# johanna-rock/quantization_analysis

Measured on AMD Instinct MI355X. Metric: 32x32 tiles/s for mixed-tile-greedy (bf16->BFP{8,4,2}); achieved HBM GB/s vs peak, higher is better.
Workload: dtype f32/f64

## Files before the change

### quantization_analysis_amd/csrc/mtq_fast.hip

```cpp
#include <hip/hip_runtime.h>
#include <stdint.h>
#include <stdlib.h>

#include "../../include/mtq.h"
#include "mtq_device.hpp"
#include "mtq_error.hpp"

namespace mtq {

typedef unsigned short us2 __attribute__((ext_vector_type(2)));
typedef short s2 __attribute__((ext_vector_type(2)));

__device__ __forceinline__ us2 as_us2(uint32_t x) { return __builtin_bit_cast(us2, x); }
__device__ __forceinline__ s2 as_s2(uint32_t x) { return __builtin_bit_cast(s2, x); }
__device__ __forceinline__ uint32_t as_u32(us2 x) { return __builtin_bit_cast(uint32_t, x); }
__device__ __forceinline__ uint32_t as_u32(s2 x) { return __builtin_bit_cast(uint32_t, x); }

#ifndef MTQ_FAST_WAVES
#define MTQ_FAST_WAVES 2
#endif
constexpr int kFastWaves = MTQ_FAST_WAVES;
constexpr int kUnitTiles = 4;
constexpr int kUnitCols = kUnitTiles * kTile;
constexpr int kInBytes = kTile * kUnitCols * 2;
// ... 315 lines not shown

__host__ __device__ constexpr int rolled_waves(uint32_t sums, uint32_t errs)
{
#ifdef MTQ_ROLLED_WAVES_PER_SIMD_FORCE
    return MTQ_ROLLED_WAVES_PER_SIMD_FORCE;
#elif defined(MTQ_K1_INTDOM)
    return (sums == 7u && errs == 7u) ? 3 : 4;
#else
    const uint32_t any = sums | errs;
    const int n = (int)((any & 1u) + ((any >> 1) & 1u) + ((any >> 2) & 1u));
    if (n >= 2) return 3;
    return errs == 0u ? 5 : 4;
#endif
}

struct PlaceArgs { uint32_t eval_mask; int o_bf16, o8, o4, o2; };
__device__ __forceinline__ void place_stat(const PlaceArgs pa, double *rec_t, int sidx, double r)
{
    if (sidx == 0) {
        rec_t[0] = r;
        if (pa.eval_mask & 1u) {
            const double z = __builtin_fabs(r) * 0.0;
            rec_t[pa.o_bf16] = r; rec_t[pa.o_bf16 + 3] = z; rec_t[pa.o_bf16 + 4] = z;
        }
    } else if (sidx == 1) {
        rec_t[1] = r;
        if (pa.eval_mask & 1u) { rec_t[pa.o_bf16 + 1] = r; rec_t[pa.o_bf16 + 2] = r; }
    } else {
        const int f = (sidx - 2) >> 2, k = (sidx - 2) & 3;
        const int o = f == 0 ? pa.o8 : (f == 1 ? pa.o4 : pa.o2);
        if (pa.eval_mask & (2u << f)) rec_t[o + k] = r;
    }
}

struct ListedArgs {
    const uint32_t *list, *n_list;
    uint32_t cap;
    uint32_t *redo, *n_redo;
    uint32_t tiles_w32;
};

template <uint32_t SUMS, uint32_t ERRS, bool XS, bool LISTED>
__global__ __launch_bounds__(kFastWaves * 64, rolled_waves(SUMS, ERRS)) void tile_stats_bf16_rolled(
    const uint16_t *__restrict__ x, int64_t stride, int64_t ld, int tiles_w, int64_t tiles, int units_w, int units_per_tensor,
    int total_units, uint32_t fmt_mask, uint32_t eval_mask, uint32_t part_mask, int rec, double *__restrict__ stats, unsigned *__restrict__ work,
    unsigned launch_id, int units_per_wave, ListedArgs la, unsigned *__restrict__ mark, int self_reset)
{
    constexpr int nsum = terms_needed(SUMS, ERRS, XS);
    constexpr int npass = (nsum + kPassMax - 1) / kPassMax, per = (nsum + npass - 1) / npass;
    constexpr int scratch_doubles = kUnitTiles * per * kScratchStride;
    static_assert((scratch_doubles + kRecDoubles) * 8 <= kHalfBytes, "reduce scratch + record image must fit in half the input image");
    extern __shared__ __attribute__((aligned(16))) unsigned char lds[];
    const int lane = threadIdx.x & 63;
    const int wave = __builtin_amdgcn_readfirstlane(threadIdx.x >> 6);
    unsigned char *in = lds + wave * kRolledWaveLds;
    const uint32_t in_addr = (uint32_t)(uintptr_t)(__attribute__((address_space(3))) unsigned char *)in;
    const uint32_t t = lane >> 4, j = lane & 15;

    uint32_t dma_off[8], dma_tile[8];
#pragma unroll
    for (int i = 0; i < 8; ++i) {
        const uint32_t rho = lane >> 4;
        const uint32_t c = (lane & 15u) ^ swz(4u * (i & 3) + rho);
        const uint32_t row = 8u * (i & 3) + 2u * rho + (uint32_t)(i >> 2);
        dma_off[i] = LISTED ? (uint32_t)(row * ld * 2) + (c & 3u) * 16u : (uint32_t)(row * ld * 2) + c * 16u;
        dma_tile[i] = c >> 2;
    }
    const uint32_t rd_row = j * 256u;
    const uint32_t c0 = (4u * t) ^ swz(j);

    const int groups = (int)min(gridDim.x, (unsigned)kWorkGroups), group = (int)(blockIdx.x % (unsigned)groups);
    unsigned *queue = LISTED ? nullptr : work + group * kWorkStride;
    uint32_t n_listed = 0u;
    if constexpr (LISTED) {
        n_listed = min(*la.n_list, la.cap);
        total_units = (int)((n_listed + 3u) >> 2);
    }
    int stride_next = (int)(blockIdx.x * kFastWaves) + wave;
    auto claim_first = [&]() -> int {
        if constexpr (LISTED) {
            const int u = stride_next;
            stride_next += (int)gridDim.x * kFastWaves;
// ... 32 lines not shown
    auto locate = [&](int u) -> Where {
        Where w{nullptr, nullptr, 0ull};
        if constexpr (LISTED) {
            const uint32_t gt = listed_tile(u, (uint32_t)lane & 3u);
            const uint32_t b = gt / (uint32_t)tiles, tt = gt - b * (uint32_t)tiles;
            const uint32_t tr = tt / la.tiles_w32, tc = tt - tr * la.tiles_w32;
            w.mine = (unsigned long long)(uintptr_t)(x + (int64_t)b * stride + ((int64_t)tr * kTile) * ld + (int64_t)tc * kTile);
        } else {
            const int b = u / units_per_tensor, r = u - b * units_per_tensor, tr = r / units_w, uc = r - tr * units_w;
            w.base = reinterpret_cast<const unsigned char *>(x + (int64_t)b * stride + ((int64_t)tr * kTile) * ld + (int64_t)uc * kUnitCols);
            w.out = stats + ((int64_t)b * tiles + (int64_t)tr * tiles_w + uc * kUnitTiles) * rec;
        }
        return w;
    };
    auto issue_rows = [&](const Where &w, int odd, uint32_t half) {
        if constexpr (LISTED) {
#pragma unroll
            for (int i = 0; i < 4; ++i) {
                const uint32_t tl = odd ? dma_tile[4 + i] : dma_tile[i], off = odd ? dma_off[4 + i] : dma_off[i];
                const unsigned lo = (unsigned)__shfl((int)(unsigned)w.mine, (int)tl, 64), hi = (unsigned)__shfl((int)(unsigned)(w.mine >> 32), (int)tl, 64);
                const unsigned long long src = (((unsigned long long)hi << 32) | lo) + off;
                glds16v(reinterpret_cast<const void *>((uintptr_t)src), half + i * 1024);
            }
        } else {
#pragma unroll
            for (int i = 0; i < 4; ++i) glds16(w.base, odd ? dma_off[4 + i] : dma_off[i], half + i * 1024);
        }
    };
    const PlaceArgs pa{eval_mask, o_bf16, o8, o4, o2};
    auto tree16 = [&](const double *row) -> double {
        double v[16];
#pragma unroll
        for (int k = 0; k < 16; ++k) v[k] = row[k];
#pragma unroll
        for (int stp = 1; stp < 16; stp <<= 1)
#pragma unroll
            for (int k = 0; k < 16; k += 2 * stp) v[k] = v[k] + v[k + stp];
        return v[0];
    };

    int left = units_per_wave > 0 ? units_per_wave : 0x7FFFFFFF;
// ... 245 lines not shown
```

### quantization_analysis_amd/csrc/mtq_scan.hip

```cpp
#include <hip/hip_runtime.h>
#include <stdint.h>

#include <atomic>
#include <type_traits>
#include <stdlib.h>
#include <mutex>

#include "../../include/mtq.h"
#include "mtq_decide.hpp"
#include "mtq_error.hpp"

namespace mtq {
namespace {

constexpr int kScanMaxTilesLds = 32768;
constexpr int kTagSlots = 16384;
constexpr int kJump = 34;

} }
__device__ unsigned long long g_scan_ticks[16];
namespace mtq { namespace {

struct U128 { uint64_t lo, hi; };
__host__ __device__ inline U128 mul128(U128 a, U128 b)
{
#if defined(__HIP_DEVICE_COMPILE__)
    const uint64_t h = __umul64hi(a.lo, b.lo);
#else
    const uint64_t h = (uint64_t)(((unsigned __int128)a.lo * b.lo) >> 64);
#endif
    return {a.lo * b.lo, h + a.lo * b.hi + a.hi * b.lo};
}
// ... 55 lines not shown
__device__ inline double ld_l2(const double *p) { return __longlong_as_double((long long)ld_l2(reinterpret_cast<const unsigned long long *>(p))); }
__device__ inline void mem_wait() { __builtin_amdgcn_s_waitcnt(0); __builtin_amdgcn_fence(__ATOMIC_ACQ_REL, "workgroup"); }

__device__ inline void compiler_fence() { asm volatile("" ::: "memory"); }
__device__ inline uint64_t below(int lane) { return lane >= 64 ? ~0ull : ((1ull << lane) - 1ull); }
__device__ inline double shfl_f64(double v, int src)
{
    const unsigned long long u = (unsigned long long)__double_as_longlong(v);
    const unsigned lo = (unsigned)__shfl((int)(unsigned)u, src, 64), hi = (unsigned)__shfl((int)(unsigned)(u >> 32), src, 64);
    return __longlong_as_double((long long)(((unsigned long long)hi << 32) | lo));
}

__device__ inline uint64_t readlane_u64(uint64_t u, int src)
{
    const unsigned lo = (unsigned)__builtin_amdgcn_readlane((int)(unsigned)u, src), hi = (unsigned)__builtin_amdgcn_readlane((int)(unsigned)(u >> 32), src);
    return ((uint64_t)hi << 32) | lo;
}

__device__ inline double readlane_f64(double v, int src) { return __longlong_as_double((long long)readlane_u64((uint64_t)__double_as_longlong(v), src)); }

struct OrderLds {
    uint16_t *p;
    __device__ uint32_t get(uint32_t i) const { return p[i]; }
    __device__ void set(uint32_t i, uint32_t v) const { p[i] = (uint16_t)v; }
    __device__ void sync() const { __builtin_amdgcn_s_waitcnt(0xC07F);  __builtin_amdgcn_fence(__ATOMIC_ACQ_REL, "workgroup"); }
    __device__ void sync_reads() const { compiler_fence(); }
    __device__ void sync_writes() const { compiler_fence(); }
};
struct OrderGlobal {
    uint32_t *p;
    __device__ uint32_t get(uint32_t i) const { return ld_l2(p + i); }
    __device__ void set(uint32_t i, uint32_t v) const { p[i] = v; }
    __device__ void sync() const { mem_wait(); }
    __device__ void sync_reads() const { mem_wait(); }
    __device__ void sync_writes() const { mem_wait(); }
};

struct Rng {
    U128 state;
    bool has32;
    uint32_t u32;
    U128 a0, c0, a1, c1;
};

#ifdef MTQ_SCAN_PROFILE
#define MTQ_SHUF_TICK(slot) do { const unsigned long long now_ = clock64(); if (blockIdx.x == 0 && lane == 0) g_scan_ticks[slot] += now_ - tick_; tick_ = now_; } while (0)
#else
#define MTQ_SHUF_TICK(slot) do { } while (0)
#endif

template <bool kSwap, typename Order>
__device__ bool wave_shuffle(Rng &r, const Order &ord, int n, uint32_t *cnt, int lane)
{
    if (n < 2) return true;
#ifdef MTQ_SCAN_PROFILE
    unsigned long long tick_ = clock64();
#endif
    int i0 = n - 1;
    int budget = 8 * n + 4096;
    while (i0 >= 1) {
        if (--budget < 0) return false;
        const uint32_t mask = 0xFFFFFFFFu >> __builtin_clz((unsigned)i0);
        const int lo = (int)(mask >> 1);
        const int pend = r.has32 ? 1 : 0;
        const U128 A = pend ? r.a1 : r.a0, C = pend ? r.c1 : r.c0;
        const U128 s = add128(mul128(A, r.state), C);
        const uint64_t o = pcg_out(s);
        const int half = (lane - pend) & 1;
        uint32_t raw = half ? (uint32_t)(o >> 32) : (uint32_t)o;
        if (pend && lane == 0) raw = r.u32;
        const uint32_t v = raw & mask;
        uint64_t okmask = __ballot((int)v <= i0 - lane);
        uint64_t amb = ~(okmask | __ballot(v > (uint32_t)i0));
        while (amb) {
            const int a = __builtin_ctzll(amb);
            const int P = __builtin_popcountll(okmask & below(a));
            const uint32_t va = (uint32_t)__builtin_amdgcn_readlane((int)v, a);
            if ((int)va <= i0 - P) okmask |= 1ull << a;
            amb &= amb - 1ull;
        }
// ... 102 lines not shown
    int32_t *status;
    int32_t *counts;
    uint32_t *order_g;
    double *delta;
    double *delta2;
    const U128 *jump_a, *jump_g;
    const unsigned char *orders;
    int phase;
    uint32_t *listed, *n_listed;
    Carry *carry;
};

constexpr int kNoOffset = 0xFF;
__device__ inline double rec_at(const double *rt, uint32_t off) { return off == (uint32_t)kNoOffset ? 0.0 : rt[off]; }

template <int kN>
__device__ inline void prefix_chain(const double *lds_d, double *lds_p, int lane, double s)
{
    double v[16], w[16];
#pragma unroll
    for (int u = 0; u < 16; ++u) v[u] = lds_d[u * 4 + lane];
#pragma unroll
    for (int i0 = 0; i0 < kN; i0 += 16) {
        if (i0 + 16 < kN) {
#pragma unroll
            for (int u = 0; u < 16; ++u) w[u] = lds_d[(i0 + 16 + u) * 4 + lane];
        }
#pragma unroll
        for (int u = 0; u < 16; ++u) { s = s + v[u]; lds_p[(i0 + u) * 4 + lane] = s; }
#pragma unroll
        for (int u = 0; u < 16; ++u) v[u] = w[u];
    }
}

__device__ inline void prefix_chain_all(const double *lds_d, double *lds_p, int col, double s)
{
    double v[16], w[16];
#pragma unroll
    for (int u = 0; u < 16; ++u) v[u] = lds_d[u * 4 + col];
#pragma unroll
    for (int i0 = 0; i0 < 64; i0 += 16) {
        if (i0 + 16 < 64) {
#pragma unroll
            for (int u = 0; u < 16; ++u) w[u] = lds_d[(i0 + 16 + u) * 4 + col];
        }
#pragma unroll
        for (int u = 0; u < 16; ++u) { s = s + v[u]; lds_p[(i0 + u) * 4 + col] = s; }
#pragma unroll
        for (int u = 0; u < 16; ++u) v[u] = w[u];
    }
}

__device__ inline bool pcc_good(double n, double mean_x, double am2, double thr, double sy, double sy2, double sxy, bool &special)
{
    const double mean_y = sy / n;
    double bm2 = sy2 - n * mean_y * mean_y;
    if (bm2 < 0.0) bm2 = 0.0;
    const double denom = __builtin_sqrt(am2 * bm2);
    special = denom == 0.0;
    const double val = (sxy - n * mean_x * mean_y) / denom;
    return val >= thr;
}

#ifdef MTQ_SCAN_PROFILE
// ... 55 lines not shown
                dd[u][2] = rt[oxy_f] - rt[(po.xy >> sh) & 0xFFu];
            }
        }
#pragma unroll
        for (int u = 0; u < 4; ++u) {
            const int k = k0 + 64 * u + lane;
            if (k < nc) {
                double *d = delta + (int64_t)k * 4;
                d[0] = dd[u][0]; d[1] = dd[u][1]; d[2] = dd[u][2]; d[3] = __longlong_as_double((long long)pv[u]);
            }
        }
    }
    mem_wait();
}

template <bool kMae, typename TileAt>
__device__ inline int visit_pass(TileAt tile_at, const double *delta, int nc, int f, int8_t *map, double *lds_d, double *lds_p, int lane, double n,
                                 double mean_x, double am2, double thr, double &Sy, double &Sy2, double &Sxy, bool &any_rej)
{
    constexpr bool mae = kMae;
    int k = 0, pk = -1;
    double pdy = 0.0, pdy2 = 0.0, pdxy = 0.0;
    int pprev = 0;
    uint32_t pt = 0;
    bool accept_mode = true;
#ifdef MTQ_SCAN_PROFILE
    unsigned long long vt_ = clock64();
#define MTQ_VISIT_TICK(slot) do { const unsigned long long now_ = clock64(); if (blockIdx.x == 0 && lane == 0) g_scan_ticks[slot] += now_ - vt_; vt_ = now_; } while (0)
#else
#define MTQ_VISIT_TICK(slot) do { } while (0)
#endif
// ... 6 lines not shown
        wprev = (int)__double_as_longlong(ld_l2(d + 3));
        wt = tile_at((uint32_t)(k0 + lane));
    };
    while (k < nc) {
        if (accept_mode && span == 64 && nc - k >= 64) {
            double c_y, c_y2, c_xy, n_y = 0.0, n_y2 = 0.0, n_xy = 0.0, f_y = 0.0, f_y2 = 0.0, f_xy = 0.0;
            int c_prev, n_prev = 0, f_prev = 0;
            uint32_t c_t, n_t = 0, f_t = 0;
            if (pk == k) { c_y = pdy; c_y2 = pdy2; c_xy = pdxy; c_prev = pprev; c_t = pt; }
            else load_window(k, c_y, c_y2, c_xy, c_prev, c_t);
            bool has_next = nc - (k + 64) >= 64;
            if (has_next) load_window(k + 64, n_y, n_y2, n_xy, n_prev, n_t);
            double *dA = lds_d, *pA = lds_p, *dB = lds_d2, *pB = lds_p2;
            dA[lane * 4 + 0] = c_y; dA[lane * 4 + 1] = c_y2; dA[lane * 4 + 2] = c_xy;
            compiler_fence();
            prefix_chain_all(dA, pA, col, col == 0 ? Sy : (col == 1 ? Sy2 : Sxy));
            compiler_fence();
            bool bailed = false;
            for (;;) {
                const bool has_far = has_next && nc - (k + 128) >= 64;
                if (has_far) load_window(k + 128, f_y, f_y2, f_xy, f_prev, f_t);
                dB[lane * 4 + 0] = n_y; dB[lane * 4 + 1] = n_y2; dB[lane * 4 + 2] = n_xy;
                compiler_fence();
                const double start = pA[63 * 4 + col];
                const double cy = pA[lane * 4 + 0], cy2 = pA[lane * 4 + 1], cxy = pA[lane * 4 + 2];
                prefix_chain_all(dB, pB, col, start);
                bool special = false;
                const bool good = mae ? cy / n <= thr : pcc_good(n, mean_x, am2, thr, cy, cy2, cxy, special);
                const uint64_t okm = __ballot(good), spm = __ballot(special);
                compiler_fence();
                if (okm != ~0ull || spm != 0ull) { bailed = true; break; }
                map[c_t] = (int8_t)f;
                Sy = readlane_f64(cy, 63); Sy2 = readlane_f64(cy2, 63); Sxy = readlane_f64(cxy, 63);
                k += 64;
                if (!has_next) break;
                c_y = n_y; c_y2 = n_y2; c_xy = n_xy; c_prev = n_prev; c_t = n_t;
                n_y = f_y; n_y2 = f_y2; n_xy = f_xy; n_prev = f_prev; n_t = f_t;
                has_next = has_far;
                double *tq = dA; dA = dB; dB = tq; tq = pA; pA = pB; pB = tq;
            }
            if (bailed) { pk = k; pdy = c_y; pdy2 = c_y2; pdxy = c_xy; pprev = c_prev; pt = c_t; }
// ... 47 lines not shown
        pk = k + m;
        pdy = pdy2 = pdxy = 0.0; pprev = 0; pt = 0;
        if (pk + lane < nc) {
            const double *d = delta + (int64_t)(pk + lane) * 4;
            pdy = ld_l2(d); pdy2 = ld_l2(d + 1); pdxy = ld_l2(d + 2);
            pprev = (int)__double_as_longlong(ld_l2(d + 3));
            pt = tile_at((uint32_t)(pk + lane));
        }
        MTQ_VISIT_TICK(8);
        double cy, cy2, cxy;
        if (accept_mode) {
            lds_d[lane * 4 + 0] = dy; lds_d[lane * 4 + 1] = dy2; lds_d[lane * 4 + 2] = dxy;
            compiler_fence();
            if (lane < 3) {
                const double s0 = lane == 0 ? Sy : (lane == 1 ? Sy2 : Sxy);
                if (span == 16) prefix_chain<16>(lds_d, lds_p, lane, s0);
                else prefix_chain<64>(lds_d, lds_p, lane, s0);
            }
            compiler_fence();
            cy = lds_p[lane * 4 + 0]; cy2 = lds_p[lane * 4 + 1]; cxy = lds_p[lane * 4 + 2];
            compiler_fence();
        } else {
            cy = Sy + dy; cy2 = Sy2 + dy2; cxy = Sxy + dxy;
        }
        MTQ_VISIT_TICK(9);
        bool special = false;
        const bool good = mae ? cy / n <= thr : pcc_good(n, mean_x, am2, thr, cy, cy2, cxy, special);
        const uint64_t act = below(m);
        const uint64_t okm = __ballot(good && active) & act, spm = __ballot(special && active) & act;
        MTQ_VISIT_TICK(10);
        int j, take = -1;
        if (accept_mode) {
// ... 10 lines not shown
            if (lane < j) map[t] = (int8_t)(prev | 0x80);
            if (j > 0) any_rej = true;
            if (j < m) { if (lane == j) map[t] = (int8_t)f; take = j; k += j + 1; if (j == 0) { accept_mode = true; span = 16; } }
            else k += m;
        }
        if (take >= 0) { Sy = readlane_f64(cy, take); Sy2 = readlane_f64(cy2, take); Sxy = readlane_f64(cxy, take); }
        MTQ_VISIT_TICK(11);
#ifdef MTQ_SCAN_PROFILE
        if (blockIdx.x == 0 && lane == 0) g_scan_ticks[15] += 1;
#endif
    }
    mem_wait();
    return 0;
}

template <bool kMae, typename Order>
__device__ __forceinline__ void scan_tensor(const ScanArgs &a, const Order &ord, int b, unsigned char *lds, int lane, int wave, bool two_waves)
{
    const int T = (int)a.tiles;
    const int rec = a.rec;
    const double *st = a.stats + (int64_t)b * a.tiles * rec;
    int8_t *map = a.maps + (int64_t)b * a.tiles;
    double *delta = a.delta + (int64_t)b * a.tiles * 4;
    double *delta2 = a.delta2 + (int64_t)b * a.tiles * 4;
    double *lds_d = reinterpret_cast<double *>(lds);
    double *lds_p = lds_d + 64 * 4;
    double *lds_i = lds_p + 64 * 4;
    uint32_t *cnt = reinterpret_cast<uint32_t *>(lds_i + 64 * 5 + 64 * 4 + 64 * 4);
    uint32_t *helper_flag = cnt + kTagSlots / 4;
    constexpr bool mae = kMae;
    const int base = a.fmt[0];
    const int *o1 = mae ? a.oab : a.oy;
    Offsets3 po;
// ... 31 lines not shown
            if (lane == 0) __hip_atomic_store(helper_flag + (p - 1), 1u, __ATOMIC_RELEASE, __HIP_MEMORY_SCOPE_WORKGROUP);
        }
        return;
    }

    int status = 0;
    bool done = false;
#ifdef MTQ_SCAN_PROFILE
    if (b == 0 && lane == 0) for (int q = 8; q < 16; ++q) g_scan_ticks[q] = 0;
    unsigned long long tick_s = clock64();
#endif
    for (int i = lane; i < kTagSlots / 4; i += 64) cnt[i] = 0u;
    compiler_fence();

    Rng r;
    U128 inc;
    double sum_x = 0.0, sum_x2 = 0.0, Sy = 0.0, Sy2 = 0.0, Sxy = 0.0;
    const double n = a.n, thr = a.thr;
    auto set_jumps = [&]() {
        const int q0 = (lane >> 1) + 1, q1 = lane >= 1 ? ((lane - 1) >> 1) + 1 : 1;
        r.a0 = a.jump_a[q0]; r.c0 = mul128(a.jump_g[q0], inc);
        r.a1 = a.jump_a[q1]; r.c1 = mul128(a.jump_g[q1], inc);
    };
    int p_begin = 1;

    if (a.phase != 2) {
        for (int t = lane; t < T; t += 64) map[t] = (int8_t)base;
        if (n_sh >= 1) { inc = hdr->inc; r.state = hdr->state[0]; r.has32 = hdr->has32[0] != 0u; r.u32 = hdr->u32[0]; }
        else { seed_pcg(a.seeds[b], r.state, inc); r.has32 = false; r.u32 = 0u; }
        set_jumps();

        const int off5[5] = {0, 1, mae ? a.oab[base] : a.oy[base], a.oy2[base], a.oxy[base]};
        auto init_sums = [&](auto nc_tag, auto ahead_tag, const int *offs) -> double {
            constexpr int kNc = decltype(nc_tag)::value, kAhead = decltype(ahead_tag)::value;
            double acc = 0.0;
            double nx[kAhead][kNc];
#pragma unroll
            for (int r = 0; r < kAhead; ++r) {
#pragma unroll
                for (int c = 0; c < kNc; ++c) nx[r][c] = 0.0;
                if (64 * r + lane < T) {
                    const double *rt = st + (int64_t)(64 * r + lane) * rec;
#pragma unroll
                    for (int c = 0; c < kNc; ++c) nx[r][c] = rec_at(rt, (uint32_t)offs[c]);
                }
// ... 4 lines not shown
                    const int t0 = t00 + 64 * r;
                    if (t0 < T) {
                        const int m = min(64, T - t0);
                        if (lane < m) {
#pragma unroll
                            for (int c = 0; c < kNc; ++c) lds_i[lane * kNc + c] = nx[r][c];
                        }
                        if (t0 + 64 * kAhead + lane < T) {
                            const double *rt = st + (int64_t)(t0 + 64 * kAhead + lane) * rec;
#pragma unroll
                            for (int c = 0; c < kNc; ++c) nx[r][c] = rec_at(rt, (uint32_t)offs[c]);
                        }
                        compiler_fence();
                        if (lane < kNc) {
                            if (m == 64) {
                                double v[16], w[16];
#pragma unroll
                                for (int u = 0; u < 16; ++u) v[u] = lds_i[u * kNc + lane];
#pragma unroll
                                for (int i0 = 0; i0 < 64; i0 += 16) {
                                    if (i0 + 16 < 64) {
#pragma unroll
                                        for (int u = 0; u < 16; ++u) w[u] = lds_i[(i0 + 16 + u) * kNc + lane];
                                    }
#pragma unroll
                                    for (int u = 0; u < 16; ++u) acc = acc + v[u];
#pragma unroll
                                    for (int u = 0; u < 16; ++u) v[u] = w[u];
                                }
                            } else {
                                for (int i = 0; i < m; ++i) acc = acc + lds_i[i * kNc + lane];
                            }
                        }
                        compiler_fence();
                    }
                }
            }
            return acc;
        };
        const bool identity_base = !mae && off5[2] == 0 && off5[3] == 1 && off5[4] == 1;
        double acc;
        if (identity_base) {
            acc = init_sums(std::integral_constant<int, 2>{}, std::integral_constant<int, 10>{}, off5);
            const double s1 = shfl_f64(acc, 1), s0 = shfl_f64(acc, 0);
            acc = lane == 0 || lane == 2 ? s0 : s1;
        } else {
            acc = init_sums(std::integral_constant<int, 5>{}, std::integral_constant<int, 4>{}, off5);
        }
        sum_x = shfl_f64(acc, 0); sum_x2 = shfl_f64(acc, 1);
        Sy = shfl_f64(acc, 2); Sy2 = shfl_f64(acc, 3); Sxy = shfl_f64(acc, 4);
    } else {
        const Carry &c = a.carry[b];
        Sy = c.Sy; Sy2 = c.Sy2; Sxy = c.Sxy; sum_x = c.sum_x; sum_x2 = c.sum_x2;
        r.state = c.state; inc = c.inc; r.has32 = c.has32 != 0u; r.u32 = c.u32;
        status = c.status; done = c.done != 0;
        set_jumps();
        p_begin = a.n_formats - 1;
    }
    const double mean_x = sum_x / n;
    double am2 = sum_x2 - n * mean_x * mean_x;
    if (am2 < 0.0) am2 = 0.0;
    MTQ_SCAN_STAMP(0);

    if (a.phase != 2) {
        bool special = false;
        const bool good = mae ? Sy / n <= thr : pcc_good(n, mean_x, am2, thr, Sy, Sy2, Sxy, special);
        if (special) status = 1;
        done = !good;
        if (n_sh == 0 && !wave_shuffle<false>(r, ord, T, cnt, lane)) status = 2;
        if (two_waves) wait_helper(1);
    }
// ... 15 lines not shown
            Pg = nullptr;
            nc = 0;
            sift_map(map, T, lane, [&](int t0, uint8_t code) {
                const bool cand = (code & 0x80u) == 0u;
                const uint64_t bm = __ballot(cand);
                if (cand) ord.set((uint32_t)(nc + __builtin_popcountll(bm & below(lane))), (uint32_t)(t0 + lane));
                nc += __builtin_popcountll(bm);
            });
            ord.sync();
            if (nc == 0) break;
            if (!wave_shuffle<true>(r, ord, nc, cnt, lane)) { status = 2; break; }
            MTQ_SCAN_STAMP(2 + 3 * (p - 1));
            gather_deltas<kMae>(st, rec, po, f, nc, delta, lane, tile_at, prev_of);
        }
        MTQ_SCAN_STAMP(3 + 3 * (p - 1));
        status = visit_pass<kMae>(tile_at, dl, nc, f, map, lds_d, lds_p, lane, n, mean_x, am2, thr, Sy, Sy2, Sxy, any_rej);
        if (use_sh) { r.state = hdr->state[p]; r.has32 = hdr->has32[p] != 0u; r.u32 = hdr->u32[p]; }
        if (any_rej) pristine = false;
        MTQ_SCAN_STAMP(4 + 3 * (p - 1));
    }
    mem_wait();

    if (a.phase == 1) {
        int nc = 0;
        if (status == 0 && !done) {
            sift_map(map, T, lane, [&](int, uint8_t code) { nc += __builtin_popcountll(__ballot((code & 0x80u) == 0u)); });
            unsigned first = 0u;
            if (lane == 0 && nc > 0) first = atomicAdd(a.n_listed, (unsigned)nc);
            first = (unsigned)__builtin_amdgcn_readfirstlane((int)first);
            int at = 0;
            if (nc > 0)
                sift_map(map, T, lane, [&](int t0, uint8_t code) {
                    const bool cand = (code & 0x80u) == 0u;
                    const uint64_t bm = __ballot(cand);
                    if (cand) a.listed[first + (unsigned)(at + __builtin_popcountll(bm & below(lane)))] = (uint32_t)((int64_t)b * T + t0 + lane);
                    at += __builtin_popcountll(bm);
                });
        }
        if (lane == 0) {
            Carry &c = a.carry[b];
            c.Sy = Sy; c.Sy2 = Sy2; c.Sxy = Sxy; c.sum_x = sum_x; c.sum_x2 = sum_x2;
            c.state = r.state; c.inc = inc; c.has32 = r.has32 ? 1u : 0u; c.u32 = r.u32;
            c.status = status; c.done = (done || nc == 0) ? 1 : 0;
        }
        return;
    }

    int per_fmt[MTQ_NUM_TILE_FORMATS] = {0, 0, 0, 0};
    sift_map(map, T, lane, [&](int t0, uint8_t raw) {
        const int t = t0 + lane;
        int code = -1;
        if (t < T) { code = (int)(raw & 0x7Fu); map[t] = (int8_t)code; }
#pragma unroll
        for (int c = 0; c < MTQ_NUM_TILE_FORMATS; ++c) per_fmt[c] += __builtin_popcountll(__ballot(code == c));
    });
    if (lane == 0) {
        a.status[b] = status;
// ... 43 lines not shown
        a.status[b] = s_nan ? 1 : 0;
        if (a.counts)
            for (int c = 0; c < MTQ_NUM_TILE_FORMATS; ++c) a.counts[b * MTQ_NUM_TILE_FORMATS + c] = s_cnt[c];
    }
}

#ifndef MTQ_SCAN_SETPRIO
#define MTQ_SCAN_SETPRIO 0
#endif
#ifdef MTQ_SCAN_WAVES_PER_EU
#define MTQ_SCAN_BUDGET __attribute__((amdgpu_waves_per_eu(MTQ_SCAN_WAVES_PER_EU, MTQ_SCAN_WAVES_PER_EU)))
#else
#define MTQ_SCAN_BUDGET
#endif

__global__ __launch_bounds__(128) MTQ_SCAN_BUDGET void greedy_scan_pcc_lds(ScanArgs a)
{
    extern __shared__ __attribute__((aligned(16))) unsigned char lds[];
    if (MTQ_SCAN_SETPRIO) __builtin_amdgcn_s_setprio(MTQ_SCAN_SETPRIO);
    const int lane = threadIdx.x & 63, wave = __builtin_amdgcn_readfirstlane((int)(threadIdx.x >> 6));
    OrderLds ord{reinterpret_cast<uint16_t *>(lds)};
    if (a.metric == MTQ_METRIC_MAE) scan_tensor<true>(a, ord, blockIdx.x, lds + 2 * ((a.tiles + 7) & ~(int64_t)7), lane, wave, blockDim.x == 128);
    else scan_tensor<false>(a, ord, blockIdx.x, lds + 2 * ((a.tiles + 7) & ~(int64_t)7), lane, wave, blockDim.x == 128);
}

__global__ __launch_bounds__(128) MTQ_SCAN_BUDGET void greedy_scan_pcc_global(ScanArgs a)
{
    extern __shared__ __attribute__((aligned(16))) unsigned char lds[];
    if (MTQ_SCAN_SETPRIO) __builtin_amdgcn_s_setprio(MTQ_SCAN_SETPRIO);
    const int lane = threadIdx.x & 63, wave = __builtin_amdgcn_readfirstlane((int)(threadIdx.x >> 6));
    OrderGlobal ord{a.order_g + (int64_t)blockIdx.x * a.tiles};
    if (a.metric == MTQ_METRIC_MAE) scan_tensor<true>(a, ord, blockIdx.x, lds, lane, wave, blockDim.x == 128);
    else scan_tensor<false>(a, ord, blockIdx.x, lds, lane, wave, blockDim.x == 128);
}

constexpr size_t kFixedLds = (64 * 4 + 64 * 4 + 64 * 5 + 64 * 4 + 64 * 4) * sizeof(double) + kTagSlots + 16;

struct OrdersArgs {
    uint64_t seed;
    int64_t tiles;
    int n_orders;
    unsigned char *out;
    const U128 *jump_a, *jump_g;
};

template <typename Order>
__device__ void make_order(const OrdersArgs &a, const Order &ord, uint32_t *cnt, uint32_t *P, int which, int lane, bool copy_out)
{
    const int T = (int)a.tiles;
    OrdersHdr *hdr = reinterpret_cast<OrdersHdr *>(a.out);
    for (int i = lane; i < kTagSlots / 4; i += 64) cnt[i] = 0u;
    compiler_fence();
    Rng r;
    U128 inc;
    seed_pcg(a.seed, r.state, inc);
    r.has32 = false;
    r.u32 = 0u;
    const int q0 = (lane >> 1) + 1, q1 = lane >= 1 ? ((lane - 1) >> 1) + 1 : 1;
    r.a0 = a.jump_a[q0]; r.c0 = mul128(a.jump_g[q0], inc);
    r.a1 = a.jump_a[q1]; r.c1 = mul128(a.jump_g[q1], inc);
    bool ok = wave_shuffle<false>(r, ord, T, cnt, lane);
    if (which == 0 && lane == 0) {
        hdr->state[0] = r.state; hdr->has32[0] = r.has32 ? 1u : 0u; hdr->u32[0] = r.u32;
        hdr->inc = inc; hdr->tiles = (uint32_t)T; hdr->n_orders = (uint32_t)a.n_orders; hdr->seed = a.seed;
    }
    if (which == 1) ok = wave_shuffle<false>(r, ord, T, cnt, lane) && ok;
    for (int t = lane; t < T; t += 64) ord.set((uint32_t)t, (uint32_t)t);
    ord.sync();
    ok = wave_shuffle<true>(r, ord, T, cnt, lane) && ok;
    ord.sync();
    if (copy_out)
        for (int t = lane; t < T; t += 64) P[t] = ord.get((uint32_t)t);
    if (lane == 0) {
        hdr->state[1 + which] = r.state; hdr->has32[1 + which] = r.has32 ? 1u : 0u; hdr->u32[1 + which] = r.u32;
        hdr->ok[which] = ok ? 1u : 0u;
    }
}

__global__ __launch_bounds__(64) void scan_orders(OrdersArgs a)
// ... 21 lines not shown
        const U128 mult = {kMultLo, kMultHi};
        h[0] = {1ull, 0ull};
        h[kJump] = {0ull, 0ull};
        for (int q = 1; q < kJump; ++q) {
            h[kJump + q] = add128(mul128(h[kJump + q - 1], mult), U128{1ull, 0ull});
            h[q] = mul128(h[q - 1], mult);
        }
        U128 *d = nullptr;
        if (hipMalloc(reinterpret_cast<void **>(&d), sizeof(h)) != hipSuccess) return nullptr;
        if (hipMemcpy(d, h, sizeof(h), hipMemcpyHostToDevice) != hipSuccess) { (void)hipFree(d); return nullptr; }
        g_jump_tab[dev] = d;
    }
    return g_jump_tab[dev];
}

std::atomic<bool> g_lds_raised[64][2];

int raise_lds(int dev, int which, const void *fn, int bytes)
{
    if (dev < 64 && g_lds_raised[dev][which].load(std::memory_order_acquire)) return MTQ_OK;
    if (hipFuncSetAttribute(fn, hipFuncAttributeMaxDynamicSharedMemorySize, bytes) != hipSuccess) return fail(MTQ_ERR_HIP, "could not raise the dynamic LDS limit");
    if (dev < 64) g_lds_raised[dev][which].store(true, std::memory_order_release);
    return MTQ_OK;
}

}
}

using namespace mtq;

void mtq::scan_shutdown()
{
    std::lock_guard<std::mutex> lock(g_jump_mu);
    for (int d = 0; d < 64; ++d) {
        if (g_jump_tab[d]) { (void)hipFree(g_jump_tab[d]); g_jump_tab[d] = nullptr; }
        g_lds_raised[d][0].store(false); g_lds_raised[d][1].store(false);
    }
}

extern "C" int mtq_debug_scan_ticks(uint64_t out[16])
{
    if (!out) return fail(MTQ_ERR_INVALID, "null argument");
    if (int rc = require_device()) return rc;
    unsigned long long h[16];
    if (hipMemcpyFromSymbol(h, HIP_SYMBOL(g_scan_ticks), sizeof(h)) != hipSuccess) return fail(MTQ_ERR_HIP, "hipMemcpyFromSymbol failed");
    for (int i = 0; i < 16; ++i) out[i] = h[i];
    return MTQ_OK;
}

extern "C" size_t mtq_greedy_scan_scratch_bytes(int64_t count, int64_t tiles)
{
// ... 85 lines not shown
    const U128 *jt = jump_tables(dev);
    if (!jt) return fail(MTQ_ERR_HIP, "could not upload the jump-ahead tables");
    a.jump_a = jt;
    a.jump_g = jt + kJump;
    a.delta = static_cast<double *>(scratch);
    a.delta2 = a.delta + (size_t)count * (size_t)tiles * 4;
    a.order_g = reinterpret_cast<uint32_t *>(static_cast<unsigned char *>(scratch) + (size_t)count * (size_t)tiles * 8 * sizeof(double));
    hipStream_t st = static_cast<hipStream_t>(stream);
    if (metric == MTQ_METRIC_ATOL) {
        hipLaunchKernelGGL(greedy_atol, dim3((unsigned)count), dim3(256), 0, st, a);
        return check_launch("mtq_greedy_scan_device");
    }
    const unsigned threads = (orders && phase != 2) ? 128u : 64u;
    static int shared_lds = -1;
    if (shared_lds < 0) { const char *e = getenv("MTQ_SCAN_SHARED_LDS"); shared_lds = e ? atoi(e) : 0; }
    if (tiles <= kScanMaxTilesLds && !(threads == 128u && !shared_lds)) {
        const size_t lds = 2 * (size_t)((tiles + 7) & ~(int64_t)7) + kFixedLds;
        if (int rc = raise_lds(dev, 0, reinterpret_cast<const void *>(greedy_scan_pcc_lds), 2 * kScanMaxTilesLds + (int)kFixedLds)) return rc;
        hipLaunchKernelGGL(greedy_scan_pcc_lds, dim3((unsigned)count), dim3(threads), lds, st, a);
    } else {
        hipLaunchKernelGGL(greedy_scan_pcc_global, dim3((unsigned)count), dim3(threads), kFixedLds, st, a);
    }
    return check_launch("mtq_greedy_scan_device");
}

extern "C" int mtq_greedy_scan_device(const double *stats, int64_t count, int64_t tiles, uint32_t fmt_mask, const int *formats, int n_formats,
                                      int metric, double threshold, double elem_count, const uint64_t *seeds, int8_t *maps, int32_t *status,
                                      int32_t *counts, void *scratch, size_t scratch_bytes, void *stream)
{
    return mtq_greedy_scan_device_ex(stats, count, tiles, fmt_mask, formats, n_formats, metric, threshold, elem_count, seeds, maps, status, counts,
                                     scratch, scratch_bytes, nullptr, 0, nullptr, nullptr, nullptr, stream);
}
```

Baseline: 1.239 billion.

## Reduce register pressure in tile-stats and scan kernels to raise occupancy

The tile-stats kernel no longer keeps precomputed DMA offset and tile arrays in registers. It recomputes per-piece chunk offsets from one base value and raises the waves-per-SIMD hint for one sums/errs combination. The greedy scan kernel gains a lean variant with shallower prefix-chain prefetch depth and a higher occupancy bound. Per-lane RNG jump constants move from persistent state to local loads, and RNG state is made wave-uniform. The lean variant is chosen when there are several tensors or a later phase, trading load latency hiding for occupancy.

```diff
diff --git a/quantization_analysis_amd/csrc/mtq_fast.hip b/quantization_analysis_amd/csrc/mtq_fast.hip
--- a/quantization_analysis_amd/csrc/mtq_fast.hip
+++ b/quantization_analysis_amd/csrc/mtq_fast.hip
@@ -353,6 +353,14 @@
 #endif
 }
 
+__host__ __device__ constexpr int rolled_cap(uint32_t sums, uint32_t errs)
+{
+#ifndef MTQ_ROLLED_WAVES_PER_SIMD_FORCE
+    if (sums == 3u && errs == 1u) return 4;
+#endif
+    return rolled_waves(sums, errs);
+}
+
 struct PlaceArgs { uint32_t eval_mask; int o_bf16, o8, o4, o2; };
 __device__ __forceinline__ void place_stat(const PlaceArgs pa, double *rec_t, int sidx, double r)
 {
@@ -380,7 +388,7 @@
 };
 
 template <uint32_t SUMS, uint32_t ERRS, bool XS, bool LISTED>
-__global__ __launch_bounds__(kFastWaves * 64, rolled_waves(SUMS, ERRS)) void tile_stats_bf16_rolled(
+__global__ __launch_bounds__(kFastWaves * 64, rolled_cap(SUMS, ERRS)) void tile_stats_bf16_rolled(
     const uint16_t *__restrict__ x, int64_t stride, int64_t ld, int tiles_w, int64_t tiles, int units_w, int units_per_tensor,
     int total_units, uint32_t fmt_mask, uint32_t eval_mask, uint32_t part_mask, int rec, double *__restrict__ stats, unsigned *__restrict__ work,
     unsigned launch_id, int units_per_wave, ListedArgs la, unsigned *__restrict__ mark, int self_reset)
@@ -396,15 +404,13 @@
     const uint32_t in_addr = (uint32_t)(uintptr_t)(__attribute__((address_space(3))) unsigned char *)in;
     const uint32_t t = lane >> 4, j = lane & 15;
 
-    uint32_t dma_off[8], dma_tile[8];
-#pragma unroll
-    for (int i = 0; i < 8; ++i) {
-        const uint32_t rho = lane >> 4;
-        const uint32_t c = (lane & 15u) ^ swz(4u * (i & 3) + rho);
-        const uint32_t row = 8u * (i & 3) + 2u * rho + (uint32_t)(i >> 2);
-        dma_off[i] = LISTED ? (uint32_t)(row * ld * 2) + (c & 3u) * 16u : (uint32_t)(row * ld * 2) + c * 16u;
-        dma_tile[i] = c >> 2;
-    }
+    const uint32_t dma_c = ((uint32_t)lane & 15u) ^ (2u * ((uint32_t)lane >> 4));
+    const uint32_t dma_row = (uint32_t)(2u * ((uint32_t)lane >> 4) * ld * 2);
+    auto piece_chunk = [&](int k) -> uint32_t {
+        uint32_t c = dma_c;
+        asm volatile("" : "+v"(c));
+        return c ^ (k == 0 ? 0u : (k == 1 ? 1u : (k == 2 ? 9u : 8u)));
+    };
     const uint32_t rd_row = j * 256u;
     const uint32_t c0 = (4u * t) ^ swz(j);
 
@@ -467,17 +473,20 @@
         return w;
     };
     auto issue_rows = [&](const Where &w, int odd, uint32_t half) {
+        const uint32_t row0 = (uint32_t)(odd * ld * 2);
+        const uint32_t row8 = (uint32_t)(8 * ld * 2);
         if constexpr (LISTED) {
 #pragma unroll
             for (int i = 0; i < 4; ++i) {
-                const uint32_t tl = odd ? dma_tile[4 + i] : dma_tile[i], off = odd ? dma_off[4 + i] : dma_off[i];
+                const uint32_t c = piece_chunk(i);
+                const uint32_t tl = c >> 2, off = dma_row + (row0 + (uint32_t)i * row8) + (c & 3u) * 16u;
                 const unsigned lo = (unsigned)__shfl((int)(unsigned)w.mine, (int)tl, 64), hi = (unsigned)__shfl((int)(unsigned)(w.mine >> 32), (int)tl, 64);
                 const unsigned long long src = (((unsigned long long)hi << 32) | lo) + off;
                 glds16v(reinterpret_cast<const void *>((uintptr_t)src), half + i * 1024);
             }
         } else {
 #pragma unroll
-            for (int i = 0; i < 4; ++i) glds16(w.base, odd ? dma_off[4 + i] : dma_off[i], half + i * 1024);
+            for (int i = 0; i < 4; ++i) glds16(w.base, dma_row + (row0 + (uint32_t)i * row8) + piece_chunk(i) * 16u, half + i * 1024);
         }
     };
     const PlaceArgs pa{eval_mask, o_bf16, o8, o4, o2};
diff --git a/quantization_analysis_amd/csrc/mtq_scan.hip b/quantization_analysis_amd/csrc/mtq_scan.hip
--- a/quantization_analysis_amd/csrc/mtq_scan.hip
+++ b/quantization_analysis_amd/csrc/mtq_scan.hip
@@ -16,6 +16,8 @@
 constexpr int kScanMaxTilesLds = 32768;
 constexpr int kTagSlots = 16384;
 constexpr int kJump = 34;
+constexpr int kChainDeep = 16;
+constexpr int kChainLean = 4;
 
 } }
 __device__ unsigned long long g_scan_ticks[16];
@@ -101,6 +103,12 @@
 __device__ inline uint64_t readlane_u64(uint64_t u, int src)
 {
     const unsigned lo = (unsigned)__builtin_amdgcn_readlane((int)(unsigned)u, src), hi = (unsigned)__builtin_amdgcn_readlane((int)(unsigned)(u >> 32), src);
+    return ((uint64_t)hi << 32) | lo;
+}
+
+__device__ inline uint64_t uniform_u64(uint64_t u)
+{
+    const unsigned lo = (unsigned)__builtin_amdgcn_readfirstlane((int)(unsigned)u), hi = (unsigned)__builtin_amdgcn_readfirstlane((int)(unsigned)(u >> 32));
     return ((uint64_t)hi << 32) | lo;
 }
 
@@ -123,11 +131,14 @@
     __device__ void sync_writes() const { mem_wait(); }
 };
 
+__device__ inline U128 uniform_u128(U128 u) { return {uniform_u64(u.lo), uniform_u64(u.hi)}; }
+
 struct Rng {
     U128 state;
     bool has32;
     uint32_t u32;
-    U128 a0, c0, a1, c1;
+    U128 inc;
+    const U128 *jump_a, *jump_g;
 };
 
 #ifdef MTQ_SCAN_PROFILE
@@ -143,6 +154,8 @@
 #ifdef MTQ_SCAN_PROFILE
     unsigned long long tick_ = clock64();
 #endif
+    const int q0 = (lane >> 1) + 1, q1 = lane >= 1 ? ((lane - 1) >> 1) + 1 : 1;
+    const U128 a0 = r.jump_a[q0], c0 = mul128(r.jump_g[q0], r.inc), a1 = r.jump_a[q1], c1 = mul128(r.jump_g[q1], r.inc);
     int i0 = n - 1;
     int budget = 8 * n + 4096;
     while (i0 >= 1) {
@@ -150,7 +163,7 @@
         const uint32_t mask = 0xFFFFFFFFu >> __builtin_clz((unsigned)i0);
         const int lo = (int)(mask >> 1);
         const int pend = r.has32 ? 1 : 0;
-        const U128 A = pend ? r.a1 : r.a0, C = pend ? r.c1 : r.c0;
+        const U128 A = pend ? a1 : a0, C = pend ? c1 : c0;
         const U128 s = add128(mul128(A, r.state), C);
         const uint64_t o = pcg_out(s);
         const int half = (lane - pend) & 1;
@@ -283,40 +296,41 @@
 constexpr int kNoOffset = 0xFF;
 __device__ inline double rec_at(const double *rt, uint32_t off) { return off == (uint32_t)kNoOffset ? 0.0 : rt[off]; }
 
-template <int kN>
+template <int kN, int kD>
 __device__ inline void prefix_chain(const double *lds_d, double *lds_p, int lane, double s)
 {
-    double v[16], w[16];
-#pragma unroll
-    for (int u = 0; u < 16; ++u) v[u] = lds_d[u * 4 + lane];
-#pragma unroll
-    for (int i0 = 0; i0 < kN; i0 += 16) {
-        if (i0 + 16 < kN) {
-#pragma unroll
-            for (int u = 0; u < 16; ++u) w[u] = lds_d[(i0 + 16 + u) * 4 + lane];
-        }
-#pragma unroll
-        for (int u = 0; u < 16; ++u) { s = s + v[u]; lds_p[(i0 + u) * 4 + lane] = s; }
-#pragma unroll
-        for (int u = 0; u < 16; ++u) v[u] = w[u];
-    }
-}
-
+    double v[kD], w[kD];
+#pragma unroll
+    for (int u = 0; u < kD; ++u) v[u] = lds_d[u * 4 + lane];
+#pragma unroll
+    for (int i0 = 0; i0 < kN; i0 += kD) {
+        if (i0 + kD < kN) {
+#pragma unroll
+            for (int u = 0; u < kD; ++u) w[u] = lds_d[(i0 + kD + u) * 4 + lane];
+        }
+#pragma unroll
+        for (int u = 0; u < kD; ++u) { s = s + v[u]; lds_p[(i0 + u) * 4 + lane] = s; }
+#pragma unroll
+        for (int u = 0; u < kD; ++u) v[u] = w[u];
+    }
+}
+
+template <int kD>
 __device__ inline void prefix_chain_all(const double *lds_d, double *lds_p, int col, double s)
 {
-    double v[16], w[16];
-#pragma unroll
-    for (int u = 0; u < 16; ++u) v[u] = lds_d[u * 4 + col];
-#pragma unroll
-    for (int i0 = 0; i0 < 64; i0 += 16) {
-        if (i0 + 16 < 64) {
-#pragma unroll
-            for (int u = 0; u < 16; ++u) w[u] = lds_d[(i0 + 16 + u) * 4 + col];
-        }
-#pragma unroll
-        for (int u = 0; u < 16; ++u) { s = s + v[u]; lds_p[(i0 + u) * 4 + col] = s; }
-#pragma unroll
-        for (int u = 0; u < 16; ++u) v[u] = w[u];
+    double v[kD], w[kD];
+#pragma unroll
+    for (int u = 0; u < kD; ++u) v[u] = lds_d[u * 4 + col];
+#pragma unroll
+    for (int i0 = 0; i0 < 64; i0 += kD) {
+        if (i0 + kD < 64) {
+#pragma unroll
+            for (int u = 0; u < kD; ++u) w[u] = lds_d[(i0 + kD + u) * 4 + col];
+        }
+#pragma unroll
+        for (int u = 0; u < kD; ++u) { s = s + v[u]; lds_p[(i0 + u) * 4 + col] = s; }
+#pragma unroll
+        for (int u = 0; u < kD; ++u) v[u] = w[u];
     }
 }
 
@@ -402,7 +416,7 @@
     mem_wait();
 }
 
-template <bool kMae, typename TileAt>
+template <bool kMae, int kD, typename TileAt>
 __device__ inline int visit_pass(TileAt tile_at, const double *delta, int nc, int f, int8_t *map, double *lds_d, double *lds_p, int lane, double n,
                                  double mean_x, double am2, double thr, double &Sy, double &Sy2, double &Sxy, bool &any_rej)
 {
@@ -439,7 +453,7 @@
             double *dA = lds_d, *pA = lds_p, *dB = lds_d2, *pB = lds_p2;
             dA[lane * 4 + 0] = c_y; dA[lane * 4 + 1] = c_y2; dA[lane * 4 + 2] = c_xy;
             compiler_fence();
-            prefix_chain_all(dA, pA, col, col == 0 ? Sy : (col == 1 ? Sy2 : Sxy));
+            prefix_chain_all<kD>(dA, pA, col, col == 0 ? Sy : (col == 1 ? Sy2 : Sxy));
             compiler_fence();
             bool bailed = false;
             for (;;) {
@@ -449,7 +463,7 @@
                 compiler_fence();
                 const double start = pA[63 * 4 + col];
                 const double cy = pA[lane * 4 + 0], cy2 = pA[lane * 4 + 1], cxy = pA[lane * 4 + 2];
-                prefix_chain_all(dB, pB, col, start);
+                prefix_chain_all<kD>(dB, pB, col, start);
                 bool special = false;
                 const bool good = mae ? cy / n <= thr : pcc_good(n, mean_x, am2, thr, cy, cy2, cxy, special);
                 const uint64_t okm = __ballot(good), spm = __ballot(special);
@@ -527,8 +541,8 @@
             compiler_fence();
             if (lane < 3) {
                 const double s0 = lane == 0 ? Sy : (lane == 1 ? Sy2 : Sxy);
-                if (span == 16) prefix_chain<16>(lds_d, lds_p, lane, s0);
-                else prefix_chain<64>(lds_d, lds_p, lane, s0);
+                if (span == 16) prefix_chain<16, kD>(lds_d, lds_p, lane, s0);
+                else prefix_chain<64, kD>(lds_d, lds_p, lane, s0);
             }
             compiler_fence();
             cy = lds_p[lane * 4 + 0]; cy2 = lds_p[lane * 4 + 1]; cxy = lds_p[lane * 4 + 2];
@@ -569,9 +583,10 @@
     return 0;
 }
 
-template <bool kMae, typename Order>
+template <bool kMae, bool kLean, typename Order>
 __device__ __forceinline__ void scan_tensor(const ScanArgs &a, const Order &ord, int b, unsigned char *lds, int lane, int wave, bool two_waves)
 {
+    constexpr int kD = kLean ? kChainLean : kChainDeep;
     const int T = (int)a.tiles;
     const int rec = a.rec;
     const double *st = a.stats + (int64_t)b * a.tiles * rec;
@@ -633,21 +648,16 @@
     compiler_fence();
 
     Rng r;
-    U128 inc;
+    r.jump_a = a.jump_a; r.jump_g = a.jump_g;
     double sum_x = 0.0, sum_x2 = 0.0, Sy = 0.0, Sy2 = 0.0, Sxy = 0.0;
     const double n = a.n, thr = a.thr;
-    auto set_jumps = [&]() {
-        const int q0 = (lane >> 1) + 1, q1 = lane >= 1 ? ((lane - 1) >> 1) + 1 : 1;
-        r.a0 = a.jump_a[q0]; r.c0 = mul128(a.jump_g[q0], inc);
-        r.a1 = a.jump_a[q1]; r.c1 = mul128(a.jump_g[q1], inc);
-    };
     int p_begin = 1;
 
     if (a.phase != 2) {
         for (int t = lane; t < T; t += 64) map[t] = (int8_t)base;
-        if (n_sh >= 1) { inc = hdr->inc; r.state = hdr->state[0]; r.has32 = hdr->has32[0] != 0u; r.u32 = hdr->u32[0]; }
-        else { seed_pcg(a.seeds[b], r.state, inc); r.has32 = false; r.u32 = 0u; }
-        set_jumps();
+        if (n_sh >= 1) { r.inc = hdr->inc; r.state = hdr->state[0]; r.has32 = hdr->has32[0] != 0u; r.u32 = hdr->u32[0]; }
+        else { seed_pcg(a.seeds[b], r.state, r.inc); r.has32 = false; r.u32 = 0u; }
+        r.state = uniform_u128(r.state); r.inc = uniform_u128(r.inc); r.u32 = (uint32_t)__builtin_amdgcn_readfirstlane((int)r.u32);
 
         const int off5[5] = {0, 1, mae ? a.oab[base] : a.oy[base], a.oy2[base], a.oxy[base]};
         auto init_sums = [&](auto nc_tag, auto ahead_tag, const int *offs) -> double {
@@ -682,19 +692,19 @@
                         compiler_fence();
                         if (lane < kNc) {
                             if (m == 64) {
-                                double v[16], w[16];
-#pragma unroll
-                                for (int u = 0; u < 16; ++u) v[u] = lds_i[u * kNc + lane];
-#pragma unroll
-                                for (int i0 = 0; i0 < 64; i0 += 16) {
-                                    if (i0 + 16 < 64) {
-#pragma unroll
-                                        for (int u = 0; u < 16; ++u) w[u] = lds_i[(i0 + 16 + u) * kNc + lane];
+                                double v[kD], w[kD];
+#pragma unroll
+                                for (int u = 0; u < kD; ++u) v[u] = lds_i[u * kNc + lane];
+#pragma unroll
+                                for (int i0 = 0; i0 < 64; i0 += kD) {
+                                    if (i0 + kD < 64) {
+#pragma unroll
+                                        for (int u = 0; u < kD; ++u) w[u] = lds_i[(i0 + kD + u) * kNc + lane];
                                     }
 #pragma unroll
-                                    for (int u = 0; u < 16; ++u) acc = acc + v[u];
-#pragma unroll
-                                    for (int u = 0; u < 16; ++u) v[u] = w[u];
+                                    for (int u = 0; u < kD; ++u) acc = acc + v[u];
+#pragma unroll
+                                    for (int u = 0; u < kD; ++u) v[u] = w[u];
                                 }
                             } else {
                                 for (int i = 0; i < m; ++i) acc = acc + lds_i[i * kNc + lane];
@@ -720,9 +730,9 @@
     } else {
         const Carry &c = a.carry[b];
         Sy = c.Sy; Sy2 = c.Sy2; Sxy = c.Sxy; sum_x = c.sum_x; sum_x2 = c.sum_x2;
-        r.state = c.state; inc = c.inc; r.has32 = c.has32 != 0u; r.u32 = c.u32;
+        r.state = c.state; r.inc = c.inc; r.has32 = c.has32 != 0u; r.u32 = c.u32;
+        r.state = uniform_u128(r.state); r.inc = uniform_u128(r.inc); r.u32 = (uint32_t)__builtin_amdgcn_readfirstlane((int)r.u32);
         status = c.status; done = c.done != 0;
-        set_jumps();
         p_begin = a.n_formats - 1;
     }
     const double mean_x = sum_x / n;
@@ -768,8 +778,8 @@
             gather_deltas<kMae>(st, rec, po, f, nc, delta, lane, tile_at, prev_of);
         }
         MTQ_SCAN_STAMP(3 + 3 * (p - 1));
-        status = visit_pass<kMae>(tile_at, dl, nc, f, map, lds_d, lds_p, lane, n, mean_x, am2, thr, Sy, Sy2, Sxy, any_rej);
-        if (use_sh) { r.state = hdr->state[p]; r.has32 = hdr->has32[p] != 0u; r.u32 = hdr->u32[p]; }
+        status = visit_pass<kMae, kD>(tile_at, dl, nc, f, map, lds_d, lds_p, lane, n, mean_x, am2, thr, Sy, Sy2, Sxy, any_rej);
+        if (use_sh) { r.state = uniform_u128(hdr->state[p]); r.has32 = hdr->has32[p] != 0u; r.u32 = (uint32_t)__builtin_amdgcn_readfirstlane((int)hdr->u32[p]); }
         if (any_rej) pristine = false;
         MTQ_SCAN_STAMP(4 + 3 * (p - 1));
     }
@@ -794,7 +804,7 @@
         if (lane == 0) {
             Carry &c = a.carry[b];
             c.Sy = Sy; c.Sy2 = Sy2; c.Sxy = Sxy; c.sum_x = sum_x; c.sum_x2 = sum_x2;
-            c.state = r.state; c.inc = inc; c.has32 = r.has32 ? 1u : 0u; c.u32 = r.u32;
+            c.state = r.state; c.inc = r.inc; c.has32 = r.has32 ? 1u : 0u; c.u32 = r.u32;
             c.status = status; c.done = (done || nc == 0) ? 1 : 0;
         }
         return;
@@ -868,24 +878,26 @@
 #define MTQ_SCAN_BUDGET
 #endif
 
-__global__ __launch_bounds__(128) MTQ_SCAN_BUDGET void greedy_scan_pcc_lds(ScanArgs a)
+template <bool kLean>
+__global__ __launch_bounds__(128, kLean ? 4 : 1) MTQ_SCAN_BUDGET void greedy_scan_pcc_lds(ScanArgs a)
 {
     extern __shared__ __attribute__((aligned(16))) unsigned char lds[];
     if (MTQ_SCAN_SETPRIO) __builtin_amdgcn_s_setprio(MTQ_SCAN_SETPRIO);
     const int lane = threadIdx.x & 63, wave = __builtin_amdgcn_readfirstlane((int)(threadIdx.x >> 6));
     OrderLds ord{reinterpret_cast<uint16_t *>(lds)};
-    if (a.metric == MTQ_METRIC_MAE) scan_tensor<true>(a, ord, blockIdx.x, lds + 2 * ((a.tiles + 7) & ~(int64_t)7), lane, wave, blockDim.x == 128);
-    else scan_tensor<false>(a, ord, blockIdx.x, lds + 2 * ((a.tiles + 7) & ~(int64_t)7), lane, wave, blockDim.x == 128);
-}
-
-__global__ __launch_bounds__(128) MTQ_SCAN_BUDGET void greedy_scan_pcc_global(ScanArgs a)
+    if (a.metric == MTQ_METRIC_MAE) scan_tensor<true, kLean>(a, ord, blockIdx.x, lds + 2 * ((a.tiles + 7) & ~(int64_t)7), lane, wave, blockDim.x == 128);
+    else scan_tensor<false, kLean>(a, ord, blockIdx.x, lds + 2 * ((a.tiles + 7) & ~(int64_t)7), lane, wave, blockDim.x == 128);
+}
+
+template <bool kLean>
+__global__ __launch_bounds__(128, kLean ? 4 : 1) MTQ_SCAN_BUDGET void greedy_scan_pcc_global(ScanArgs a)
 {
     extern __shared__ __attribute__((aligned(16))) unsigned char lds[];
     if (MTQ_SCAN_SETPRIO) __builtin_amdgcn_s_setprio(MTQ_SCAN_SETPRIO);
     const int lane = threadIdx.x & 63, wave = __builtin_amdgcn_readfirstlane((int)(threadIdx.x >> 6));
     OrderGlobal ord{a.order_g + (int64_t)blockIdx.x * a.tiles};
-    if (a.metric == MTQ_METRIC_MAE) scan_tensor<true>(a, ord, blockIdx.x, lds, lane, wave, blockDim.x == 128);
-    else scan_tensor<false>(a, ord, blockIdx.x, lds, lane, wave, blockDim.x == 128);
+    if (a.metric == MTQ_METRIC_MAE) scan_tensor<true, kLean>(a, ord, blockIdx.x, lds, lane, wave, blockDim.x == 128);
+    else scan_tensor<false, kLean>(a, ord, blockIdx.x, lds, lane, wave, blockDim.x == 128);
 }
 
 constexpr size_t kFixedLds = (64 * 4 + 64 * 4 + 64 * 5 + 64 * 4 + 64 * 4) * sizeof(double) + kTagSlots + 16;
@@ -906,17 +918,14 @@
     for (int i = lane; i < kTagSlots / 4; i += 64) cnt[i] = 0u;
     compiler_fence();
     Rng r;
-    U128 inc;
-    seed_pcg(a.seed, r.state, inc);
+    r.jump_a = a.jump_a; r.jump_g = a.jump_g;
+    seed_pcg(a.seed, r.state, r.inc);
     r.has32 = false;
     r.u32 = 0u;
-    const int q0 = (lane >> 1) + 1, q1 = lane >= 1 ? ((lane - 1) >> 1) + 1 : 1;
-    r.a0 = a.jump_a[q0]; r.c0 = mul128(a.jump_g[q0], inc);
-    r.a1 = a.jump_a[q1]; r.c1 = mul128(a.jump_g[q1], inc);
     bool ok = wave_shuffle<false>(r, ord, T, cnt, lane);
     if (which == 0 && lane == 0) {
         hdr->state[0] = r.state; hdr->has32[0] = r.has32 ? 1u : 0u; hdr->u32[0] = r.u32;
-        hdr->inc = inc; hdr->tiles = (uint32_t)T; hdr->n_orders = (uint32_t)a.n_orders; hdr->seed = a.seed;
+        hdr->inc = r.inc; hdr->tiles = (uint32_t)T; hdr->n_orders = (uint32_t)a.n_orders; hdr->seed = a.seed;
     }
     if (which == 1) ok = wave_shuffle<false>(r, ord, T, cnt, lane) && ok;
     for (int t = lane; t < T; t += 64) ord.set((uint32_t)t, (uint32_t)t);
@@ -968,7 +977,7 @@
     return g_jump_tab[dev];
 }
 
-std::atomic<bool> g_lds_raised[64][2];
+std::atomic<bool> g_lds_raised[64][3];
 
 int raise_lds(int dev, int which, const void *fn, int bytes)
 {
@@ -988,7 +997,7 @@
     std::lock_guard<std::mutex> lock(g_jump_mu);
     for (int d = 0; d < 64; ++d) {
         if (g_jump_tab[d]) { (void)hipFree(g_jump_tab[d]); g_jump_tab[d] = nullptr; }
-        g_lds_raised[d][0].store(false); g_lds_raised[d][1].store(false);
+        for (int k = 0; k < 3; ++k) g_lds_raised[d][k].store(false);
     }
 }
 
@@ -1104,12 +1113,18 @@
     const unsigned threads = (orders && phase != 2) ? 128u : 64u;
     static int shared_lds = -1;
     if (shared_lds < 0) { const char *e = getenv("MTQ_SCAN_SHARED_LDS"); shared_lds = e ? atoi(e) : 0; }
+    static int lean_env = -2;
+    if (lean_env == -2) { const char *e = getenv("MTQ_SCAN_LEAN"); lean_env = e && *e ? (atoi(e) != 0 ? 1 : 0) : -1; }
+    const bool lean = lean_env >= 0 ? lean_env == 1 : (count > 1 || phase != 0);
     if (tiles <= kScanMaxTilesLds && !(threads == 128u && !shared_lds)) {
         const size_t lds = 2 * (size_t)((tiles + 7) & ~(int64_t)7) + kFixedLds;
-        if (int rc = raise_lds(dev, 0, reinterpret_cast<const void *>(greedy_scan_pcc_lds), 2 * kScanMaxTilesLds + (int)kFixedLds)) return rc;
-        hipLaunchKernelGGL(greedy_scan_pcc_lds, dim3((unsigned)count), dim3(threads), lds, st, a);
+        const void *fn = lean ? reinterpret_cast<const void *>(greedy_scan_pcc_lds<true>) : reinterpret_cast<const void *>(greedy_scan_pcc_lds<false>);
+        if (int rc = raise_lds(dev, lean ? 2 : 0, fn, 2 * kScanMaxTilesLds + (int)kFixedLds)) return rc;
+        if (lean) hipLaunchKernelGGL(greedy_scan_pcc_lds<true>, dim3((unsigned)count), dim3(threads), lds, st, a);
+        else hipLaunchKernelGGL(greedy_scan_pcc_lds<false>, dim3((unsigned)count), dim3(threads), lds, st, a);
     } else {
-        hipLaunchKernelGGL(greedy_scan_pcc_global, dim3((unsigned)count), dim3(threads), kFixedLds, st, a);
+        if (lean) hipLaunchKernelGGL(greedy_scan_pcc_global<true>, dim3((unsigned)count), dim3(threads), kFixedLds, st, a);
+        else hipLaunchKernelGGL(greedy_scan_pcc_global<false>, dim3((unsigned)count), dim3(threads), kFixedLds, st, a);
     }
     return check_launch("mtq_greedy_scan_device");
 }
```

After: 1.144 billion. -7.6%, worse.
